# owkin/PyDESeq2

Measured on AMD Instinct MI355X. Metric: genes/sec end-to-end deseq2() (size factors->dispersion->IRLS->Wald), higher is better.
Workload: dtype f64

## Files before the change

### pydeseq2_amd/csrc/dsq_k_stats.hip

```cpp
#include <cfloat>
#include <hip/hip_cooperative_groups.h>

#include <cstdio>

#include "dsq_dispatch.h"
#include "dsq_launch.h"
#include "dsq_stats.h"
#include "dsq_trend.h"

namespace dsq {

struct LdsSorter {
    __device__ __forceinline__ static void wave_sync() {
        __builtin_amdgcn_fence(__ATOMIC_RELEASE, "wavefront");
        __builtin_amdgcn_wave_barrier();
        __builtin_amdgcn_fence(__ATOMIC_ACQUIRE, "wavefront");
    }
    __device__ __forceinline__ int operator()(double* buf, int n) const {
        int L = 1;
        while (L < n) L <<= 1;
        const int lane = threadIdx.x & 63;
        for (int k = n + lane; k < L; k += 64) buf[k] = INFINITY;
        wave_sync();
        for (int k = 2; k <= L; k <<= 1) {
// ... 53 lines not shown
    }
    if (CHECK && isbad) atomicOr(bad, 1);
}

template <class SrcT, class DstT, bool CHECK>
__global__ __launch_bounds__(256) void k_repitch(const SrcT* __restrict__ src, int N, int G,
                                                 DstT* __restrict__ dst, int ldn, int* bad) {
    const int g = blockIdx.x;
    int isbad = 0;
    for (int n = blockIdx.y * 256 + threadIdx.x; n < N; n += gridDim.y * 256) {
        const SrcT v = src[(size_t)g * N + n];
        if (CHECK) {
            if ((double)v < 0.0 || (double)v > 2147483647.0) isbad = 1;
        }
        dst[(size_t)g * ldn + n] = (DstT)v;
    }
    if (CHECK && isbad) atomicOr(bad, 1);
}

__global__ __launch_bounds__(256) void k_widen_u16(const uint16_t* __restrict__ src, int32_t* __restrict__ dst, size_t n) {
    const size_t n8 = n / 8;
    for (size_t i = (size_t)blockIdx.x * 256 + threadIdx.x; i < n8; i += (size_t)gridDim.x * 256) {
        const uint4 v = ((const uint4*)src)[i];
        int4 a, b;
        a.x = (int)(v.x & 0xffffu); a.y = (int)(v.x >> 16); a.z = (int)(v.y & 0xffffu); a.w = (int)(v.y >> 16);
        b.x = (int)(v.z & 0xffffu); b.y = (int)(v.z >> 16); b.z = (int)(v.w & 0xffffu); b.w = (int)(v.w >> 16);
        ((int4*)dst)[2 * i] = a;
        ((int4*)dst)[2 * i + 1] = b;
    }
    for (size_t i = n8 * 8 + (size_t)blockIdx.x * 256 + threadIdx.x; i < n; i += (size_t)gridDim.x * 256) dst[i] = (int)src[i];
}
hipError_t launch_widen_u16(hipStream_t st, const uint16_t* src, int32_t* dst, size_t n) {
    if (n == 0) return hipSuccess;
    size_t blocks = (n / 8 + 255) / 256;
    if (blocks > 4096) blocks = 4096;
    if (blocks < 1) blocks = 1;
    hipLaunchKernelGGL(k_widen_u16, dim3((unsigned)blocks), dim3(256), 0, st, src, dst, n);
    return hipGetLastError();
}

hipError_t launch_transpose_counts(hipStream_t st, const void* src, int count_type, int layout, int N,
                                   int G, int32_t* dst, int ldn, int* bad_flag) {
    if (N <= 0 || G <= 0) return hipSuccess;
    if (layout == 0) {
        const dim3 grid((G + 63) / 64, (N + 63) / 64), block(256);
        if (count_type == 1)
            hipLaunchKernelGGL((k_transpose<int64_t, int32_t, true>), grid, block, 0, st,
                               (const int64_t*)src, N, G, dst, ldn, bad_flag);
        else
            hipLaunchKernelGGL((k_transpose<int32_t, int32_t, true>), grid, block, 0, st,
                               (const int32_t*)src, N, G, dst, ldn, bad_flag);
    } else {
        const dim3 grid(G, (N + 255) / 256 > 64 ? 64 : (N + 255) / 256), block(256);
        if (count_type == 1)
            hipLaunchKernelGGL((k_repitch<int64_t, int32_t, true>), grid, block, 0, st,
                               (const int64_t*)src, N, G, dst, ldn, bad_flag);
        else
            hipLaunchKernelGGL((k_repitch<int32_t, int32_t, true>), grid, block, 0, st,
                               (const int32_t*)src, N, G, dst, ldn, bad_flag);
    }
    return hipGetLastError();
}

hipError_t launch_transpose_f64(hipStream_t st, const double* src, int layout, int N, int G,
                                double* dst, int ldn) {
    if (N <= 0 || G <= 0) return hipSuccess;
    if (layout == 0) {
        const dim3 grid((G + 63) / 64, (N + 63) / 64), block(256);
        hipLaunchKernelGGL((k_transpose<double, double, false>), grid, block, 0, st, src, N, G, dst, ldn,
                           (int*)nullptr);
    } else {
        const dim3 grid(G, (N + 255) / 256 > 64 ? 64 : (N + 255) / 256), block(256);
        hipLaunchKernelGGL((k_repitch<double, double, false>), grid, block, 0, st, src, N, G, dst, ldn,
                           (int*)nullptr);
    }
    return hipGetLastError();
}

__global__ __launch_bounds__(kBlock) void k_logmeans(const int32_t* __restrict__ y, int ldn, int N,
                                                     int G, double* __restrict__ logmeans,
                                                     uint8_t* __restrict__ nonzero) {
    __shared__ double s_logint[256];
    static_assert(kBlock == 256, "one table entry per thread");
    s_logint[threadIdx.x] = kLogInt[threadIdx.x];
    __syncthreads();
    const int g = blockIdx.x * kWavesPerBlock + (threadIdx.x >> 6);
    if (g >= G) return;
    double lm;
    int nz;
    gene_logmean<DeviceWave>(y + (size_t)g * ldn, N, lm, nz, s_logint);
    if ((threadIdx.x & 63) == 0) {
        logmeans[g] = lm;
        nonzero[g] = (uint8_t)nz;
    }
}

__global__ __launch_bounds__(kBlock) void k_logmeans_pos(const int32_t* __restrict__ y, int ldn, int N, int G,
                                                         double* __restrict__ logmeans,
                                                         uint8_t* __restrict__ usable) {
    const int g = blockIdx.x * kWavesPerBlock + (threadIdx.x >> 6);
    if (g >= G) return;
    const int32_t* yr = y + (size_t)g * ldn;
    double s = 0.0;
    for (int n = threadIdx.x & 63; n < N; n += 64) {
        const int v = yr[n];
        if (v != 0) s += log_count(v);
    }
    s = DeviceWave::sum(s) / (double)N;
    if ((threadIdx.x & 63) == 0) {
        logmeans[g] = s;
        usable[g] = (uint8_t)((s > 0.0 && s != INFINITY) ? 1 : 0);
    }
}

hipError_t launch_logmeans_pos(hipStream_t st, const int32_t* y, int ldn, int N, int G, double* logmeans,
                               uint8_t* usable) {
    if (G <= 0) return hipSuccess;
    hipLaunchKernelGGL(k_logmeans_pos, dim3(genes_to_blocks(G)), dim3(kBlock), 0, st, y, ldn, N, G, logmeans, usable);
    return hipGetLastError();
}

hipError_t launch_logmeans(hipStream_t st, const int32_t* y, int ldn, int N, int G, double* logmeans,
                           uint8_t* nonzero) {
    if (G <= 0) return hipSuccess;
    hipLaunchKernelGGL(k_logmeans, dim3(genes_to_blocks(G)), dim3(kBlock), 0, st, y, ldn, N, G, logmeans,
                       nonzero);
    return hipGetLastError();
}

__device__ __forceinline__ unsigned long long f64_key(double v) {
    const unsigned long long b = (unsigned long long)__double_as_longlong(v);
    return (b & 0x8000000000000000ull) ? ~b : (b | 0x8000000000000000ull);
}
__device__ __forceinline__ double key_f64(unsigned long long k) {
    const unsigned long long b = (k & 0x8000000000000000ull) ? (k & 0x7fffffffffffffffull) : ~k;
    return __longlong_as_double((long long)b);
}

template <class SrcT>
__global__ __launch_bounds__(256) void k_ratio_keys(const SrcT* __restrict__ counts, int N, int G,
                                                    const double* __restrict__ logmeans,
                                                    const uint8_t* __restrict__ mask,
                                                    unsigned long long* __restrict__ keys) {
    const int n = blockIdx.y;
    for (int g = blockIdx.x * 256 + threadIdx.x; g < G; g += gridDim.x * 256) {
        const double lm = logmeans[g];
        const bool use = (lm != -INFINITY) && (lm == lm) && (mask == nullptr || mask[g] != 0);
        unsigned long long k = ~0ull;
        const double c = (double)counts[(size_t)n * G + g];
        if (use && c > 0.0) k = f64_key((c < 256.0 ? kLogInt[(int)c] : flog(c)) - lm);
        keys[(size_t)n * G + g] = k;
    }
}

struct MedianShared {
    unsigned int hist[2][2048];
    unsigned long long prefix[2];
    unsigned int rank[2];
    unsigned int M;
};

__device__ __forceinline__ int pick_digit(const unsigned int* h, int nbins, unsigned int& r) {
    const int lane = threadIdx.x & 63;
    const int per = nbins / 64;
    unsigned int mine = 0;
    for (int k = 0; k < per; ++k) mine += h[lane * per + k];
    unsigned int incl = mine;
#pragma unroll
    for (int o = 1; o < 64; o <<= 1) {
        const unsigned int v = __shfl_up(incl, o, 64);
        if (lane >= o) incl += v;
    }
    const unsigned int excl = incl - mine;
    const bool here = (excl <= r) && (r < incl);
    const unsigned long long ball = __ballot(here);
    const int src = ball ? (__ffsll((long long)ball) - 1) : 63;
    int d = nbins - 1;
    unsigned int rr = 0;
    if (lane == src) {
        unsigned int acc = excl;
        int k = 0;
        for (; k < per - 1; ++k) {
            const unsigned int c = h[lane * per + k];
            if (acc + c > r) break;
            acc += c;
        }
        d = lane * per + k;
        rr = r - acc;
    }
    d = __shfl(d, src, 64);
    r = __shfl(rr, src, 64);
    return d;
}

template <class Each>
__device__ void block_median_each(Each each, MedianShared& S, double& median, unsigned int& M_out) {
    const int shifts[6] = {53, 42, 31, 20, 9, 0};
    const int tid = threadIdx.x, NT = blockDim.x;
    for (int pass = 0; pass < 6; ++pass) {
        const int shift = shifts[pass];
        const int nbins = pass == 5 ? 512 : 2048;
        for (int i = tid; i < 2 * 2048; i += NT) (&S.hist[0][0])[i] = 0;
        __syncthreads();
        const unsigned long long p0 = S.prefix[0], p1 = S.prefix[1];
        const unsigned long long himask = pass == 0 ? 0ull : (~0ull << (shifts[pass - 1]));
        each([&](unsigned long long k) {
            if (k == ~0ull) return;
            const unsigned int d = (unsigned int)(k >> shift) & (unsigned int)(nbins - 1);
            if (pass == 0) {
                atomicAdd(&S.hist[0][d], 1u);
            } else {
                if ((k & himask) == p0) atomicAdd(&S.hist[0][d], 1u);
                if ((k & himask) == p1) atomicAdd(&S.hist[1][d], 1u);
            }
        });
        __syncthreads();
        if (pass == 0) {
            if (tid < 64) {
                unsigned int c = 0;
                for (int k = tid; k < 2048; k += 64) c += S.hist[0][k];
#pragma unroll
                for (int o = 32; o >= 1; o >>= 1) c += __shfl_xor(c, o, 64);
                if (tid == 0) {
                    S.M = c;
                    S.rank[0] = c ? (c - 1) / 2 : 0;
                    S.rank[1] = c / 2;
                    S.prefix[0] = 0ull;
                    S.prefix[1] = 0ull;
                }
            }
            __syncthreads();
        }
        const int w = tid >> 6;
        if (w < 2) {
            unsigned int r = S.rank[w];
            const int d = pick_digit(S.hist[pass == 0 ? 0 : w], nbins, r);
            if ((tid & 63) == 0) {
                S.rank[w] = r;
                S.prefix[w] |= ((unsigned long long)d << shift);
            }
        }
        __syncthreads();
    }
    const unsigned int M = S.M;
    M_out = M;
    if (M == 0) { median = NAN; return; }
    const double v0 = key_f64(S.prefix[0]), v1 = key_f64(S.prefix[1]);
    median = ((M - 1) / 2 == M / 2) ? v0 : (v0 + v1) / 2.0;
}

template <class KeyFn>
__device__ void block_median(KeyFn key, int n, MedianShared& S, double& median, unsigned int& M_out) {
    block_median_each(
        [&](auto fn) {
            for (int i = threadIdx.x; i < n; i += blockDim.x) fn(key(i));
        },
        S, median, M_out);
}

__global__ __launch_bounds__(1024) void k_row_median(const unsigned long long* __restrict__ keys, int N,
                                                     int G, double* __restrict__ sf) {
    __shared__ MedianShared S;
    const int n = blockIdx.x;
    const unsigned long long* row = keys + (size_t)n * G;
    double med;
    unsigned int M;
    block_median([&](int g) { return row[g]; }, G, S, med, M);
    if (threadIdx.x == 0) sf[n] = (M == 0) ? NAN : exp(med);
}

constexpr int kSelCand = 1024;

struct ValueSelectShared {
    unsigned int hist[2048];
    double cand[kSelCand];
    double dred[16][2];
    unsigned int ured[16][2];
    unsigned int wtot[16];
    unsigned int bin[2], pre[2], ncand;
    double a[2];
};

__device__ __forceinline__ void vs_block_reduce(ValueSelectShared& S, double& lo, double& hi, unsigned int& c0,
                                                unsigned int& c1) {
#pragma unroll
    for (int o = 32; o >= 1; o >>= 1) {
        lo = dmin(lo, __shfl_xor(lo, o, 64));
        hi = dmax(hi, __shfl_xor(hi, o, 64));
        c0 += __shfl_xor(c0, o, 64);
        c1 += __shfl_xor(c1, o, 64);
    }
    const int w = threadIdx.x >> 6;
    __syncthreads();
    if ((threadIdx.x & 63) == 0) { S.dred[w][0] = lo; S.dred[w][1] = hi; S.ured[w][0] = c0; S.ured[w][1] = c1; }
    __syncthreads();
    lo = S.dred[0][0]; hi = S.dred[0][1]; c0 = S.ured[0][0]; c1 = S.ured[0][1];
    for (int q = 1; q < (int)(blockDim.x >> 6); ++q) {
        lo = dmin(lo, S.dred[q][0]); hi = dmax(hi, S.dred[q][1]);
        c0 += S.ured[q][0]; c1 += S.ured[q][1];
    }
}

template <int NT, class Each>
__device__ void block_median_values(Each each, ValueSelectShared& S, double& median, unsigned int& M_out) {
    const int tid = threadIdx.x, lane = tid & 63, w = tid >> 6;
    double lo = INFINITY, hi = -INFINITY;
    unsigned int n_fin = 0, n_low = 0, n_high = 0, none = 0;
    each([&](double x) {
        if (x != x) return;
        if (x == -INFINITY) { n_low += 1; return; }
        if (x == INFINITY) { n_high += 1; return; }
        lo = dmin(lo, x); hi = dmax(hi, x);
        n_fin += 1;
    });
    vs_block_reduce(S, lo, hi, n_fin, n_low);
    {
        double d0 = 0.0, d1 = 0.0;
        vs_block_reduce(S, d0, d1, n_high, none);
    }
    const unsigned int M = n_fin + n_low + n_high;
    M_out = M;
    if (M == 0) { median = NAN; return; }
    const unsigned int r0 = (M - 1) / 2, r1 = M / 2;
    if (r1 < n_low) { median = -INFINITY; return; }
    if (r1 >= n_low + n_fin) { median = (r0 < n_low) ? NAN : INFINITY; return; }
    const bool low0 = r0 < n_low;
    unsigned int q0 = (low0 ? r1 : r0) - n_low, q1 = r1 - n_low;
    unsigned int cnt = n_fin;
    double a0 = NAN, a1 = NAN;
    for (int level = 0; level < 64; ++level) {
        if (lo == hi) { a0 = lo; a1 = lo; break; }
        const double scale = 2048.0 / (hi - lo);
        auto bin_of = [&](double x) {
            const int bb = (int)((x - lo) * scale);
            return bb > 2047 ? 2047 : bb;
        };
        const bool direct = cnt <= (unsigned int)kSelCand;
        int b0 = 0, b1 = 2047;
        if (!direct) {
            for (int i = tid; i < 2048; i += NT) S.hist[i] = 0;
            __syncthreads();
            each([&](double x) {
                if (x >= lo && x <= hi) atomicAdd(&S.hist[bin_of(x)], 1u);
            });
            __syncthreads();
            {
                constexpr int PER = 2048 / NT;
                unsigned int h[PER], all = 0;
#pragma unroll
                for (int q = 0; q < PER; ++q) { h[q] = S.hist[PER * tid + q]; all += h[q]; }
                unsigned int incl = all;
#pragma unroll
                for (int o = 1; o < 64; o <<= 1) {
                    const unsigned int t = __shfl_up(incl, o, 64);
                    if (lane >= o) incl += t;
                }
                if (lane == 63) S.wtot[w] = incl;
                __syncthreads();
                unsigned int base = 0;
                for (int q = 0; q < w; ++q) base += S.wtot[q];
                unsigned int excl = base + incl - all;
#pragma unroll
                for (int q = 0; q < PER; ++q) {
#pragma unroll
                    for (int which = 0; which < 2; ++which) {
                        const unsigned int t = which ? q1 : q0;
                        if (excl <= t && t < excl + h[q]) { S.bin[which] = PER * tid + q; S.pre[which] = excl; }
                    }
                    excl += h[q];
                }
                __syncthreads();
            }
            b0 = (int)S.bin[0]; b1 = (int)S.bin[1];
            const unsigned int pre0 = S.pre[0];
            const unsigned int c0 = S.hist[b0], csel = c0 + (b1 != b0 ? S.hist[b1] : 0u);
            q0 -= pre0; q1 -= pre0;
            if (csel > (unsigned int)kSelCand) {
                double nlo = INFINITY, nhi = -INFINITY, lo1 = INFINITY;
                unsigned int d0 = 0, d1 = 0;
                each([&](double x) {
                    if (x >= lo && x <= hi) {
                        const int bb = bin_of(x);
                        if (bb == b0) { nlo = dmin(nlo, x); nhi = dmax(nhi, x); }
                        if (bb == b1) lo1 = dmin(lo1, x);
                    }
                });
                if (b0 != b1) {
                    vs_block_reduce(S, lo1, nhi, d0, d1);
                    a0 = nhi; a1 = lo1;
                    break;
                }
                vs_block_reduce(S, nlo, nhi, d0, d1);
                lo = nlo; hi = nhi; cnt = c0;
                continue;
            }
        }
        if (tid == 0) { S.ncand = 0; S.a[0] = NAN; S.a[1] = NAN; }
        __syncthreads();
        each([&](double x) {
            if (x >= lo && x <= hi) {
                bool take = direct;
                if (!direct) {
                    const int bb = bin_of(x);
                    take = bb == b0 || bb == b1;
                }
                if (take) S.cand[atomicAdd(&S.ncand, 1u)] = x;
            }
        });
        __syncthreads();
        const unsigned int m = S.ncand;
        for (int i = tid; i < (int)m; i += NT) {
            const double c = S.cand[i];
            unsigned int less = 0, eq = 0;
            for (unsigned int j = 0; j < m; ++j) {
                const double cj = S.cand[j];
                less += cj < c;
                eq += cj == c;
            }
            if (less <= q0 && q0 < less + eq) S.a[0] = c;
            if (less <= q1 && q1 < less + eq) S.a[1] = c;
        }
        __syncthreads();
        a0 = S.a[0]; a1 = S.a[1];
        break;
    }
    const double v0 = low0 ? -INFINITY : a0;
    median = (r0 == r1) ? v0 : (v0 + a1) / 2.0;
    __syncthreads();
}

__global__ void k_prior_res(const double* __restrict__ gw_raw, const double* __restrict__ fitted, int n,
                            double min_disp, double max_disp, double* __restrict__ res) {
    const int i = blockIdx.x * blockDim.x + threadIdx.x;
    if (i >= n) return;
    const double g = dmin(dmax(gw_raw[i], min_disp), max_disp);
    res[i] = (g >= 100.0 * min_disp) ? log(g) - log(fitted[i]) : NAN;
}

__global__ __launch_bounds__(1024) void k_prior_mad(const double* __restrict__ res, int n, double* __restrict__ out) {
    __shared__ ValueSelectShared S;
    const int tid = threadIdx.x;
    double center, mad;
    unsigned int M, M2;
    auto walk = [&](auto&& f) {
        int i = tid;
        for (; i + 7 * 1024 < n; i += 8 * 1024) {
            double x[8];
#pragma unroll
            for (int q = 0; q < 8; ++q) x[q] = res[i + q * 1024];
#pragma unroll
            for (int q = 0; q < 8; ++q) f(x[q]);
        }
        for (; i < n; i += 1024) f(res[i]);
    };
    block_median_values<1024>([&](auto fn) { walk(fn); }, S, center, M);
    block_median_values<1024>([&](auto fn) { walk([&](double r) { fn(fabs(r - center)); }); }, S, mad, M2);
    if (tid == 0) {
        const double m = mad / 0.67448975019608171;
        out[0] = m * m;
        out[1] = (double)M;
    }
}

size_t prior_mad_work_doubles(int n) { return (size_t)n + 8; }

hipError_t launch_prior_mad(hipStream_t st, const double* gw_raw, const double* fitted, int n, double min_disp,
                            double max_disp, double* res_scratch, double* out2) {
    if (n > 0)
        hipLaunchKernelGGL(k_prior_res, dim3((n + 255) / 256), dim3(256), 0, st, gw_raw, fitted, n, min_disp, max_disp,
                           res_scratch);
    hipLaunchKernelGGL(k_prior_mad, dim3(1), dim3(1024), 0, st, (const double*)res_scratch, n, out2);
    return hipGetLastError();
}

__global__ __launch_bounds__(256) void k_sf_compact(const double* __restrict__ logmeans,
                                                    const uint8_t* __restrict__ mask, int G,
                                                    int* __restrict__ idx, int* __restrict__ count) {
    const int g = blockIdx.x * blockDim.x + threadIdx.x;
    bool use = false;
    if (g < G) {
        const double lm = logmeans[g];
        use = (lm != -INFINITY) && (lm == lm) && (mask == nullptr || mask[g] != 0);
    }
    const unsigned long long b = __ballot(use);
    const int lane = threadIdx.x & 63;
    int base = 0;
    if (lane == 0 && b) base = atomicAdd(count, __popcll(b));
    base = __shfl(base, 0, 64);
    if (use) idx[base + __popcll(b & ((1ull << lane) - 1ull))] = g;
}

constexpr int kSfRegGenes = 32768;

template <class SrcT, int NT, int kSfRegKeys>
__global__ __launch_bounds__(NT) void k_sf_row(const SrcT* __restrict__ counts, int N, int G,
                                                 const double* __restrict__ logmeans, const int* __restrict__ idx,
                                                 const int* __restrict__ count, double* __restrict__ sf,
                                                 int zeros_low) {
    __shared__ ValueSelectShared S;
    const int tid = threadIdx.x;
    const int n = blockIdx.x, Gu = *count;
    if (Gu > NT * kSfRegKeys) return;
    double v[kSfRegKeys];
#pragma unroll
    for (int k = 0; k < kSfRegKeys; ++k) v[k] = NAN;
    const int kmax = (Gu + NT - 1) / NT;
    {
#pragma unroll
        for (int k0 = 0; k0 < kSfRegKeys; k0 += 8) {
            if (k0 >= kmax) continue;
            __builtin_amdgcn_sched_barrier(0);
            int g[8];
            double c[8], lm[8], tl[8];
#pragma unroll
            for (int kk = 0; kk < 8; ++kk) {
                const int j = tid + (k0 + kk) * NT;
                g[kk] = idx[j < Gu ? j : Gu - 1];
            }
#pragma unroll
            for (int kk = 0; kk < 8; ++kk) {
                c[kk] = (double)counts[(size_t)n * G + g[kk]];
                lm[kk] = logmeans[g[kk]];
            }
#pragma unroll
            for (int kk = 0; kk < 8; ++kk) tl[kk] = kLogInt[c[kk] < 256.0 ? (c[kk] > 0.0 ? (int)c[kk] : 1) : 255];
#pragma unroll
            for (int kk = 0; kk < 8; ++kk) {
                const bool in = tid + (k0 + kk) * NT < Gu, pos = c[kk] > 0.0;
                const double x = (c[kk] < 256.0 ? tl[kk] : flog(pos ? c[kk] : 1.0)) - lm[kk];
                const bool fin = in && pos, low = in && !pos && zeros_low != 0;
                v[k0 + kk] = fin ? x : (low ? -INFINITY : NAN);
            }
        }
    }
    double med;
    unsigned int M;
    block_median_values<NT>(
        [&](auto fn) {
#pragma unroll
            for (int k = 0; k < kSfRegKeys; ++k)
                if (k < kmax) fn(v[k]);
        },
        S, med, M);
    if (tid == 0) sf[n] = (M == 0) ? NAN : exp(med);
}

template <class SrcT>
__global__ __launch_bounds__(256) void k_ratio_keys_c(const SrcT* __restrict__ counts, int N, int G,
                                                      const double* __restrict__ logmeans,
                                                      const int* __restrict__ idx, const int* __restrict__ count,
                                                      unsigned long long* __restrict__ keys, int zeros_low,
                                                      int after_sf_row) {
    const int n = blockIdx.y, Gu = *count;
    if (after_sf_row && Gu <= kSfRegGenes) return;
    const unsigned long long kz = zeros_low ? f64_key(-INFINITY) : ~0ull;
    for (int j = blockIdx.x * 256 + threadIdx.x; j < Gu; j += gridDim.x * 256) {
        const int g = idx[j];
        const double c = (double)counts[(size_t)n * G + g];
        keys[(size_t)n * Gu + j] = (c > 0.0) ? f64_key((c < 256.0 ? kLogInt[(int)c] : flog(c)) - logmeans[g]) : kz;
    }
}

__global__ __launch_bounds__(1024) void k_row_median_c(const unsigned long long* __restrict__ keys, int N,
                                                       const int* __restrict__ count, double* __restrict__ sf) {
    __shared__ MedianShared S;
    const int n = blockIdx.x, Gu = *count;
    if (Gu <= kSfRegGenes) return;
    const unsigned long long* row = keys + (size_t)n * Gu;
    double med;
    unsigned int M;
    block_median([&](int g) { return row[g]; }, Gu, S, med, M);
    if (threadIdx.x == 0) sf[n] = (M == 0) ? NAN : exp(med);
}

size_t size_factors_work_doubles(int N, int G) { return (size_t)N * G + (size_t)G / 2 + 8; }

hipError_t launch_size_factors(hipStream_t st, const void* counts_sm, int count_type, int N, int G,
                               const double* logmeans, const uint8_t* gene_mask, double* work,
                               double* sf, int zeros_low) {
    if (N <= 0 || G <= 0) return hipSuccess;
    unsigned long long* keys = (unsigned long long*)work;
    int* idx = (int*)(work + (size_t)N * G);
    int* count = idx + G;
    hipError_t e0 = hipMemsetAsync(count, 0, sizeof(int), st);
    if (e0 != hipSuccess) return e0;
    hipLaunchKernelGGL(k_sf_compact, dim3((G + 255) / 256), dim3(256), 0, st, logmeans, gene_mask, G, idx, count);
    if (G <= 256 * 32) {
        if (count_type == 1)
            hipLaunchKernelGGL((k_sf_row<int64_t, 256, 32>), dim3(N), dim3(256), 0, st, (const int64_t*)counts_sm, N, G,
                               logmeans, (const int*)idx, (const int*)count, sf, zeros_low);
        else
            hipLaunchKernelGGL((k_sf_row<int32_t, 256, 32>), dim3(N), dim3(256), 0, st, (const int32_t*)counts_sm, N, G,
                               logmeans, (const int*)idx, (const int*)count, sf, zeros_low);
        return hipGetLastError();
    }
    if (count_type == 1)
        hipLaunchKernelGGL((k_sf_row<int64_t, 1024, 32>), dim3(N), dim3(1024), 0, st, (const int64_t*)counts_sm, N, G,
                           logmeans, (const int*)idx, (const int*)count, sf, zeros_low);
    else
        hipLaunchKernelGGL((k_sf_row<int32_t, 1024, 32>), dim3(N), dim3(1024), 0, st, (const int32_t*)counts_sm, N, G,
                           logmeans, (const int*)idx, (const int*)count, sf, zeros_low);
    if (G <= kSfRegGenes) return hipGetLastError();
    int gx = (G + 255) / 256 > 256 ? 256 : (G + 255) / 256;
    if (gx > 4096 / N + 1) gx = 4096 / N + 1;
    if (count_type == 1)
        hipLaunchKernelGGL((k_ratio_keys_c<int64_t>), dim3(gx, N), dim3(256), 0, st, (const int64_t*)counts_sm, N, G,
                           logmeans, (const int*)idx, (const int*)count, keys, zeros_low, 1);
    else
        hipLaunchKernelGGL((k_ratio_keys_c<int32_t>), dim3(gx, N), dim3(256), 0, st, (const int32_t*)counts_sm, N, G,
                           logmeans, (const int*)idx, (const int*)count, keys, zeros_low, 1);
    hipLaunchKernelGGL(k_row_median_c, dim3(N), dim3(1024), 0, st, (const unsigned long long*)keys, N,
                       (const int*)count, sf);
    return hipGetLastError();
}

__global__ void k_mean_inv(const double* __restrict__ sf, int N, double* out) {
    __shared__ double part[256];
    double s = 0.0;
    for (int n = threadIdx.x; n < N; n += 256) s += 1.0 / sf[n];
    part[threadIdx.x] = s;
    __syncthreads();
    for (int k = 128; k > 0; k >>= 1) {
        if (threadIdx.x < k) part[threadIdx.x] += part[threadIdx.x + k];
        __syncthreads();
    }
    if (threadIdx.x == 0) out[0] = part[0] / (double)N;
}

constexpr int kMomGenes = 4;
static inline int mom_blocks(int G) { return (G + kWavesPerBlock * kMomGenes - 1) / (kWavesPerBlock * kMomGenes); }

template <int P>
__global__ __launch_bounds__(kBlock) void k_mom(const int32_t* __restrict__ y, int ldn,
                                                const double* __restrict__ sf,
                                                const double* __restrict__ Xt,
                                                const double* __restrict__ pinvXt, int ldx, int N, int G,
                                                const double* __restrict__ s_mean_inv, double min_disp,
                                                double max_disp, double* __restrict__ normed_mean,
                                                double* __restrict__ rough, double* __restrict__ moments,
                                                double* __restrict__ mom) {
    const int g0 = (blockIdx.x * kWavesPerBlock + (threadIdx.x >> 6)) * kMomGenes;
    if (g0 >= G) return;
    const int nv = G - g0 < kMomGenes ? G - g0 : kMomGenes;
    MomOut o[kMomGenes];
    mom_lin_mu_block<DeviceWave, P, kMomGenes>(y + (size_t)g0 * ldn, ldn, nv, sf, Xt, pinvXt, ldx, N, s_mean_inv[0],
                                               min_disp, max_disp, 0.0, nullptr, nullptr, o);
    if ((threadIdx.x & 63) == 0) {
#pragma unroll
        for (int k = 0; k < kMomGenes; ++k) {
            if (k < nv) {
                normed_mean[g0 + k] = o[k].normed_mean;
                if (rough) rough[g0 + k] = o[k].rough;
                if (moments) moments[g0 + k] = o[k].moments;
                mom[g0 + k] = o[k].mom;
            }
        }
    }
}

hipError_t launch_mom(hipStream_t st, const int32_t* y, int ldn, const double* sf, const double* Xt,
                      const double* pinvXt, int ldx, int N, int G, int P_, double min_disp,
                      double max_disp, double* normed_mean, double* rough, double* moments,
                      double* mom, double* d_scalar, const double* sf_moments) {
    if (G <= 0) return hipSuccess;
    hipLaunchKernelGGL(k_mean_inv, dim3(1), dim3(256), 0, st, sf_moments ? sf_moments : sf, N, d_scalar);
    if (P_ > DSQ_REG_MAX_P)
        return launch_wide_mom(st, y, ldn, sf, Xt, pinvXt, ldx, N, G, P_, min_disp, max_disp, 0.5, normed_mean, rough,
                               moments, mom, nullptr, nullptr, d_scalar);
    const dim3 grid(mom_blocks(G)), block(kBlock);
    DSQ_DISPATCH_P(P_, hipLaunchKernelGGL(k_mom<P>, grid, block, 0, st, y, ldn, sf, Xt, pinvXt, ldx, N, G,
                                          (const double*)d_scalar, min_disp, max_disp, normed_mean, rough,
                                          moments, mom))
    return hipGetLastError();
}

template <int P>
__global__ __launch_bounds__(kBlock) void k_mom_lin_mu(const int32_t* __restrict__ y, int ldn,
                                                       const double* __restrict__ sf,
                                                       const double* __restrict__ Xt,
                                                       const double* __restrict__ pinvXt, int ldx, int N, int G,
                                                       const double* __restrict__ s_mean_inv, double min_disp,
                                                       double max_disp, double min_mu,
                                                       double* __restrict__ normed_mean, double* __restrict__ mom,
                                                       double* __restrict__ mu, double* __restrict__ coef) {
    const int g0 = (blockIdx.x * kWavesPerBlock + (threadIdx.x >> 6)) * kMomGenes;
    if (g0 >= G) return;
    const int nv = G - g0 < kMomGenes ? G - g0 : kMomGenes;
    MomOut o[kMomGenes];
    mom_lin_mu_block<DeviceWave, P, kMomGenes>(y + (size_t)g0 * ldn, ldn, nv, sf, Xt, pinvXt, ldx, N, s_mean_inv[0],
                                               min_disp, max_disp, min_mu, mu ? mu + (size_t)g0 * ldn : nullptr,
                                               coef ? coef + (size_t)g0 * P : nullptr, o);
    if ((threadIdx.x & 63) == 0) {
#pragma unroll
        for (int k = 0; k < kMomGenes; ++k) {
            if (k < nv) {
                normed_mean[g0 + k] = o[k].normed_mean;
                mom[g0 + k] = o[k].mom;
            }
        }
    }
}

hipError_t launch_mom_lin_mu(hipStream_t st, const int32_t* y, int ldn, const double* sf, const double* Xt,
                             const double* pinvXt, int ldx, int N, int G, int P_, double min_disp, double max_disp,
                             double min_mu, double* normed_mean, double* mom, double* mu, double* d_scalar,
                             double* coef) {
    if (G <= 0) return hipSuccess;
    hipLaunchKernelGGL(k_mean_inv, dim3(1), dim3(256), 0, st, sf, N, d_scalar);
    if (P_ > DSQ_REG_MAX_P)
        return launch_wide_mom(st, y, ldn, sf, Xt, pinvXt, ldx, N, G, P_, min_disp, max_disp, min_mu, normed_mean,
                               nullptr, nullptr, mom, mu, coef, d_scalar);
    const dim3 grid(mom_blocks(G)), block(kBlock);
    DSQ_DISPATCH_P(P_, hipLaunchKernelGGL(k_mom_lin_mu<P>, grid, block, 0, st, y, ldn, sf, Xt, pinvXt, ldx, N, G,
                                          (const double*)d_scalar, min_disp, max_disp, min_mu, normed_mean, mom, mu,
                                          coef))
    return hipGetLastError();
}

template <int P>
__global__ __launch_bounds__(kBlock) void k_lin_mu(const int32_t* __restrict__ y, int ldn,
                                                   const double* __restrict__ sf,
                                                   const double* __restrict__ Xt,
                                                   const double* __restrict__ pinvXt, int ldx, int N,
                                                   int G, double min_mu, double* __restrict__ mu) {
    const int g = blockIdx.x * kWavesPerBlock + (threadIdx.x >> 6);
    if (g >= G) return;
    lin_mu_gene<DeviceWave, P>(y + (size_t)g * ldn, sf, Xt, pinvXt, ldx, N, min_mu, mu + (size_t)g * ldn);
}

hipError_t launch_lin_mu(hipStream_t st, const int32_t* y, int ldn, const double* sf, const double* Xt,
                         const double* pinvXt, int ldx, int N, int G, int P_, double min_mu,
                         double* mu) {
    if (G <= 0) return hipSuccess;
    if (P_ > DSQ_REG_MAX_P) {
        return launch_wide_mom(st, y, ldn, sf, Xt, pinvXt, ldx, N, G, P_, 1e-8, 1.0, min_mu, nullptr, nullptr, nullptr,
                               nullptr, mu, nullptr, sf);
    }
    const dim3 grid(genes_to_blocks(G)), block(kBlock);
    DSQ_DISPATCH_P(P_, hipLaunchKernelGGL(k_lin_mu<P>, grid, block, 0, st, y, ldn, sf, Xt, pinvXt, ldx, N,
                                          G, min_mu, mu))
    return hipGetLastError();
}

template <int P, bool EXP = false>
__global__ __launch_bounds__(kBlock) void k_mu_from_coef(const double* __restrict__ coef, const double* __restrict__ sf,
                                                         const double* __restrict__ Xt, int ldx, int N, double min_mu,
                                                         const int32_t* __restrict__ list, int n_list,
                                                         double* __restrict__ dst, int ldn, int32_t* __restrict__ idx_out,
                                                         const int32_t* __restrict__ n_dev) {
    const int k = blockIdx.x * kWavesPerBlock + (threadIdx.x >> 6);
    if (n_dev != nullptr) n_list = min(n_list, *n_dev);
    if (k >= n_list) return;
    const int g = list[k];
    double b[P];
#pragma unroll
    for (int j = 0; j < P; ++j) b[j] = coef[(size_t)g * P + j];
    for (int n = blockIdx.y * 64 + DeviceWave::lane(); n < N; n += 64 * gridDim.y) {
        double yh = 0.0;
#pragma unroll
        for (int j = 0; j < P; ++j) yh += Xt[j * ldx + n] * b[j];
        dst[(size_t)k * ldn + n] = EXP ? sf[n] * exp(yh) : dmax(sf[n] * yh, min_mu);
    }
    if ((threadIdx.x & 63) == 0 && blockIdx.y == 0) idx_out[k] = k;
}
static inline unsigned mu_row_slices(int N) {
    const int s = (N + 255) / 256;
    return (unsigned)(s < 1 ? 1 : (s > 16 ? 16 : s));
}

hipError_t launch_mu_from_coef(hipStream_t st, const double* coef, const double* sf, const double* Xt, int ldx, int N,
                               int P_, double min_mu, const int32_t* list, int n_list, double* dst, int ldn,
                               int32_t* idx_out, const int32_t* n_dev) {
    if (n_list <= 0) return hipSuccess;
    DSQ_DISPATCH_P(P_, hipLaunchKernelGGL(k_mu_from_coef<P>, dim3(genes_to_blocks(n_list), mu_row_slices(N)), dim3(kBlock), 0, st, coef,
// ... 1103 lines not shown
```

Before: 10.76 million.

## Hold prior-MAD residuals in registers and LDS across median passes

Adds a single-block kernel for the prior-dispersion MAD that loads the residuals once into per-thread registers (32 per thread) and dynamic LDS slots. Every radix/bisection pass of both medians then rereads from on-chip storage instead of global memory, and the absolute deviations are computed in place. The counting lambda in the median is also made branch-free and the function force-inlined. The new path applies only when n is at most 65536, otherwise the old streaming kernel runs. The costs are heavy register pressure and large LDS use in a single-block kernel that runs once per fit.

```diff
diff --git a/pydeseq2_amd/csrc/dsq_k_stats.hip b/pydeseq2_amd/csrc/dsq_k_stats.hip
--- a/pydeseq2_amd/csrc/dsq_k_stats.hip
+++ b/pydeseq2_amd/csrc/dsq_k_stats.hip
@@ -379,16 +379,15 @@
 }
 
 template <int NT, class Each>
-__device__ void block_median_values(Each each, ValueSelectShared& S, double& median, unsigned int& M_out) {
+__device__ __forceinline__ void block_median_values(Each each, ValueSelectShared& S, double& median, unsigned int& M_out) {
     const int tid = threadIdx.x, lane = tid & 63, w = tid >> 6;
     double lo = INFINITY, hi = -INFINITY;
     unsigned int n_fin = 0, n_low = 0, n_high = 0, none = 0;
     each([&](double x) {
-        if (x != x) return;
-        if (x == -INFINITY) { n_low += 1; return; }
-        if (x == INFINITY) { n_high += 1; return; }
-        lo = dmin(lo, x); hi = dmax(hi, x);
-        n_fin += 1;
+        const bool low = x == -INFINITY, high = x == INFINITY;
+        const bool fin = x == x && !low && !high;
+        n_low += low; n_high += high; n_fin += fin;
+        if (fin) { lo = dmin(lo, x); hi = dmax(hi, x); }
     });
     vs_block_reduce(S, lo, hi, n_fin, n_low);
     {
@@ -539,6 +538,76 @@
     }
 }
 
+constexpr int kMadRegs = 32;
+constexpr int kMadLdsBatch = 4;
+constexpr int kMadLdsSlots = 16;
+constexpr int kMadWalk = 8;
+constexpr int kMadHeldN = 65536;
+static_assert(kMadLdsSlots % kMadLdsBatch == 0, "whole batches");
+static_assert(sizeof(ValueSelectShared) + (size_t)kMadLdsSlots * 1024 * sizeof(double) <= 160 * 1024, "one CU's LDS");
+
+__global__ __launch_bounds__(1024) void k_prior_mad_held(const double* __restrict__ res, int n, int lds_slots,
+                                                         double* __restrict__ out) {
+    __shared__ ValueSelectShared S;
+    extern __shared__ double mad_lds[];
+    const int tid = threadIdx.x;
+    double x[kMadRegs];
+#pragma unroll
+    for (int q = 0; q < kMadRegs; ++q) {
+        const int i = tid + q * 1024;
+        x[q] = (i < n) ? res[i] : NAN;
+    }
+    for (int k = 0; k < lds_slots; k += kMadLdsBatch) {
+        double t[kMadLdsBatch];
+#pragma unroll
+        for (int q = 0; q < kMadLdsBatch; ++q) {
+            const int i = tid + (kMadRegs + k + q) * 1024;
+            t[q] = (i < n) ? res[i] : NAN;
+        }
+#pragma unroll
+        for (int q = 0; q < kMadLdsBatch; ++q) mad_lds[(k + q) * 1024 + tid] = t[q];
+    }
+    const int held_n = (kMadRegs + lds_slots) * 1024;
+    auto held = [&](auto&& f, auto&& g) {
+#pragma unroll
+        for (int q = 0; q < kMadRegs; ++q)
+            if (q * 1024 < n) {
+                double v = x[q];
+                asm volatile("" : "+v"(v));
+                f(v);
+            }
+        for (int k = 0; k < lds_slots; k += kMadLdsBatch) {
+            double t[kMadLdsBatch];
+#pragma unroll
+            for (int q = 0; q < kMadLdsBatch; ++q) t[q] = mad_lds[(k + q) * 1024 + tid];
+#pragma unroll
+            for (int q = 0; q < kMadLdsBatch; ++q) f(t[q]);
+        }
+        for (int b = held_n; b < n; b += kMadWalk * 1024) {
+            double t[kMadWalk];
+#pragma unroll
+            for (int q = 0; q < kMadWalk; ++q) {
+                const int i = tid + b + q * 1024;
+                t[q] = (i < n) ? res[i] : NAN;
+            }
+#pragma unroll
+            for (int q = 0; q < kMadWalk; ++q) f(g(t[q]));
+        }
+    };
+    double center, mad;
+    unsigned int M, M2;
+    block_median_values<1024>([&](auto fn) { held(fn, [](double r) { return r; }); }, S, center, M);
+#pragma unroll
+    for (int q = 0; q < kMadRegs; ++q) x[q] = fabs(x[q] - center);
+    for (int k = 0; k < lds_slots; ++k) mad_lds[k * 1024 + tid] = fabs(mad_lds[k * 1024 + tid] - center);
+    block_median_values<1024>([&](auto fn) { held(fn, [&](double r) { return fabs(r - center); }); }, S, mad, M2);
+    if (tid == 0) {
+        const double m = mad / 0.67448975019608171;
+        out[0] = m * m;
+        out[1] = (double)M;
+    }
+}
+
 size_t prior_mad_work_doubles(int n) { return (size_t)n + 8; }
 
 hipError_t launch_prior_mad(hipStream_t st, const double* gw_raw, const double* fitted, int n, double min_disp,
@@ -546,7 +615,20 @@
     if (n > 0)
         hipLaunchKernelGGL(k_prior_res, dim3((n + 255) / 256), dim3(256), 0, st, gw_raw, fitted, n, min_disp, max_disp,
                            res_scratch);
-    hipLaunchKernelGGL(k_prior_mad, dim3(1), dim3(1024), 0, st, (const double*)res_scratch, n, out2);
+    const bool walk = getenv("DSQ_PRIOR_MAD_WALK") != nullptr;
+    if (n > kMadHeldN || walk) {
+        hipLaunchKernelGGL(k_prior_mad, dim3(1), dim3(1024), 0, st, (const double*)res_scratch, n, out2);
+        return hipGetLastError();
+    }
+    const int slots_needed = (n + 1023) / 1024 - kMadRegs;
+    int lds_slots = slots_needed > 0 ? (slots_needed + kMadLdsBatch - 1) / kMadLdsBatch * kMadLdsBatch : 0;
+    if (lds_slots > kMadLdsSlots) lds_slots = kMadLdsSlots;
+    const size_t dyn = (size_t)lds_slots * 1024 * sizeof(double);
+    if (sizeof(ValueSelectShared) + dyn > 48 * 1024) {
+        (void)hipFuncSetAttribute((const void*)k_prior_mad_held, hipFuncAttributeMaxDynamicSharedMemorySize, (int)dyn);
+        (void)hipGetLastError();
+    }
+    hipLaunchKernelGGL(k_prior_mad_held, dim3(1), dim3(1024), dyn, st, (const double*)res_scratch, n, lds_slots, out2);
     return hipGetLastError();
 }
 
```

Result: no change. 10.69 million (-0.6%).
